# SophieLangdon27/LDPC_SPARC

Hardware: AMD Instinct MI355X
Metric: codewords/sec (AMP+BP) at L=1024 M=512 / n=1944; BER match vs CPU ref (higher is better)
Workload: dtype f32; 1 GPU; C2: SPARC AMP, regular design, sub-sampled DCT operator w=2^20; L=1024, M=512, n=6144, t_max=25, batch_per_gpu=256, parallelism=mc-shard x1 (independent codewords per GPU, RCCL all-reduce of error counters), counter_allreduce=none, engine=split per-codeword (amp_cw2.hip)

## Files before the change

### include/ldpc_sparc_amd.h

```cpp
#ifndef LDPC_SPARC_AMD_H
#define LDPC_SPARC_AMD_H

#include <stddef.h>
#include <stdint.h>

#ifdef __cplusplus
extern "C" {
#endif

enum sg_status {
    SG_OK = 0,
    SG_ERR_INVALID = -2,
    SG_ERR_BAD_ARG = SG_ERR_INVALID,
    SG_ERR_NO_DEVICE = -3,
    SG_ERR_HIP = -4,
    SG_ERR_NOMEM = -5,
    SG_ERR_UNSUPPORTED = -6,
    SG_ERR_COMM = -7
};

enum sg_dectype { SG_SUMPROD = 0, SG_SUMPROD2 = 1, SG_MINSUM = 2 };
enum sg_precision { SG_F64 = 0, SG_F32 = 1 };

const char *sg_last_error(void);
// ... 123 lines not shown
                          const double *alpha, const double *vk, const double *vk0, const double *tau2, int B,
                          int L, int M, double sqrt_nPl, double *out);

int sumprod(double *ch, long *vdeg, long *cdeg, long *intrlv, int Nv, int Nc, int Nmsg,
            double *app, int max_itcount);
int sumprod2(double *ch, long *vdeg, long *cdeg, long *intrlv, int Nv, int Nc, int Nmsg,
             double *app, int max_itcount);
int minsum(double *ch, long *vdeg, long *cdeg, long *intrlv, int Nv, int Nc, int Nmsg,
           double *app, double correction_factor, int max_itcount);
double Lxor(double L1, double L2, int corr_flag);
double Lxfb(double *L, long dc, int corr_flag);


typedef struct sg_amp_plan sg_amp_plan;

int sg_amp_plan_create(int ndim, const double *W, int Lr, int Lc, int L, int M, int n,
                       const uint32_t *order0, const uint32_t *order1, int precision,
                       sg_amp_plan **out);
int sg_amp_plan_destroy(sg_amp_plan *p);
int sg_amp_plan_info(const sg_amp_plan *p, int *w, int *nT, int *Mr, int *Mc, int *P, int *Q);
int sg_amp_plan_engine(const sg_amp_plan *p, int B);
int sg_amp_last_decode(const sg_amp_plan *p, int *engine, int *handover_iter, int *on_companion);
int sg_amp_plan_set_cus(sg_amp_plan *p, int cus);
int sg_amp_last_pipelined(const sg_amp_plan *p, int *pipelined);

int sg_amp_decode(sg_amp_plan *p, const double *y, int B, const int32_t *true_idx, double awgn_var,
                  int t_max, double rtol, int phi_method, int32_t *map_idx, int32_t *t_final,
                  double *nmse, double *psi);
int sg_amp_decode_device(sg_amp_plan *p, const void *d_y, int B, const int32_t *d_true_idx,
                         double awgn_var, int t_max, double rtol, int phi_method,
                         int32_t *d_map_idx, int32_t *d_t_final, double *d_nmse, double *d_psi,
                         void *stream);
int sg_amp_decode_partial_device(sg_amp_plan *p, const void *d_y, int B, const int32_t *d_known_idx,
                                 const int32_t *d_true_idx, double awgn_var, int t_max, double rtol,
                                 int phi_method, int32_t *d_map_idx, int32_t *d_t_final, double *d_nmse,
                                 double *d_psi, void *stream);
int sg_amp_decode_partial(sg_amp_plan *p, const double *y, int B, const int32_t *known_idx,
                          const int32_t *true_idx, double awgn_var, int t_max, double rtol, int phi_method,
                          int32_t *map_idx, int32_t *t_final, double *nmse, double *psi);
int sg_amp_decode_bpsk_device(sg_amp_plan *p, const void *d_y, int B, const int32_t *d_true_word, double awgn_var,
                              int t_max, double rtol, int phi_method, int32_t *d_map_word, int32_t *d_t_final,
                              double *d_nmse, double *d_psi, void *stream);
int sg_amp_decode_bpsk(sg_amp_plan *p, const double *y, int B, const int32_t *true_word, double awgn_var, int t_max,
                       double rtol, int phi_method, int32_t *map_word, int32_t *t_final, double *nmse, double *psi);
int sg_amp_decode_bpsk_partial_device(sg_amp_plan *p, const void *d_y, int B, const int32_t *d_known_word,
                                      const int32_t *d_true_word, double awgn_var, int t_max, double rtol,
// ... 91 lines not shown
```

### ldpc_sparc_amd/_native.py

```python
import ctypes as ct
import os

import numpy as np

_HERE = os.path.dirname(os.path.abspath(__file__))
LIB_PATH = os.environ.get("LDPC_SPARC_AMD_LIB", os.path.join(_HERE, "_lib", "libldpc_sparc_amd.so"))

SG_SUMPROD, SG_SUMPROD2, SG_MINSUM = 0, 1, 2
SG_F64, SG_F32 = 0, 1
SG_OK, SG_ERR_INVALID, SG_ERR_NO_DEVICE, SG_ERR_HIP, SG_ERR_NOMEM, SG_ERR_UNSUPPORTED, SG_ERR_COMM = 0, -2, -3, -4, -5, -6, -7
SG_ERR_BAD_ARG = SG_ERR_INVALID
DECTYPES = {"sumprod": SG_SUMPROD, "sumprod2": SG_SUMPROD2, "minsum": SG_MINSUM}

_lib = None

dp = ct.POINTER(ct.c_double)
lp = ct.POINTER(ct.c_long)
vp = ct.c_void_p


class NativeError(RuntimeError):
    pass


# ... 33 lines not shown
    ("sg_ldpc_decode_device", ct.c_int,
     [vp, ct.c_int, ct.c_int, vp, ct.c_int, ct.c_int, ct.c_double, vp, vp, vp]),
    ("sg_ldpc_layer_check", ct.c_int, [vp, vp, vp, ct.c_int, ct.c_int, ct.c_int, ct.c_int]),
    ("sg_ldpc_decode_layered", ct.c_int,
     [vp, ct.c_int, ct.c_int, ct.c_int, vp, ct.c_int, ct.c_int, ct.c_double, vp, vp]),
    ("sg_ldpc_decode_layered_device", ct.c_int,
     [vp, ct.c_int, ct.c_int, ct.c_int, vp, ct.c_int, ct.c_int, ct.c_double, vp, vp, vp]),
    ("sg_ldpc_decode_layered_kernel", ct.c_int, [vp, ct.c_int, ct.c_int, ct.c_int, ct.c_char_p, ct.c_size_t]),
    ("sg_ldpc_codeword_errors_device", ct.c_int, [vp, ct.c_int, vp, vp, ct.c_int, vp, vp]),
    ("sg_ldpc_count_errors_device", ct.c_int,
     [vp, ct.c_int, vp, vp, vp, ct.c_int, ct.c_int, vp, vp]),
    ("sumprod", ct.c_int, [dp, lp, lp, lp, ct.c_int, ct.c_int, ct.c_int, dp, ct.c_int]),
    ("sumprod2", ct.c_int, [dp, lp, lp, lp, ct.c_int, ct.c_int, ct.c_int, dp, ct.c_int]),
    ("minsum", ct.c_int, [dp, lp, lp, lp, ct.c_int, ct.c_int, ct.c_int, dp, ct.c_double, ct.c_int]),
    ("Lxor", ct.c_double, [ct.c_double, ct.c_double, ct.c_int]),
    ("sg_amp_plan_create", ct.c_int, [ct.c_int, vp, ct.c_int, ct.c_int, ct.c_int, ct.c_int, ct.c_int,
                                      vp, vp, ct.c_int, ct.POINTER(vp)]),
    ("sg_amp_plan_destroy", ct.c_int, [vp]),
    ("sg_amp_plan_info", ct.c_int, [vp] + [ct.POINTER(ct.c_int)] * 6),
    ("sg_amp_plan_engine", ct.c_int, [vp, ct.c_int]),
    ("sg_amp_last_decode", ct.c_int, [vp, ct.POINTER(ct.c_int), ct.POINTER(ct.c_int), ct.POINTER(ct.c_int)]),
    ("sg_amp_plan_set_cus", ct.c_int, [vp, ct.c_int]),
    ("sg_amp_last_pipelined", ct.c_int, [vp, ct.POINTER(ct.c_int)]),
    ("sg_amp_decode", ct.c_int, [vp, vp, ct.c_int, vp, ct.c_double, ct.c_int, ct.c_double, ct.c_int,
                                 vp, vp, vp, vp]),
    ("sg_amp_decode_device", ct.c_int, [vp, vp, ct.c_int, vp, ct.c_double, ct.c_int, ct.c_double,
                                        ct.c_int, vp, vp, vp, vp, vp]),
    ("sg_amp_decode_partial", ct.c_int, [vp, vp, ct.c_int, vp, vp, ct.c_double, ct.c_int, ct.c_double, ct.c_int,
                                         vp, vp, vp, vp]),
    ("sg_amp_decode_partial_device", ct.c_int, [vp, vp, ct.c_int, vp, vp, ct.c_double, ct.c_int, ct.c_double,
                                                ct.c_int, vp, vp, vp, vp, vp]),
    ("sg_concat_known_sections_device", ct.c_int, [ct.c_int, vp, vp, ct.c_int, ct.c_int, ct.c_int, ct.c_int, ct.c_int,
                                                   ct.c_int, ct.c_int, vp, vp]),
    ("sg_amp_decode_bpsk", ct.c_int, [vp, vp, ct.c_int, vp, ct.c_double, ct.c_int, ct.c_double, ct.c_int,
                                      vp, vp, vp, vp]),
    ("sg_amp_decode_bpsk_device", ct.c_int, [vp, vp, ct.c_int, vp, ct.c_double, ct.c_int, ct.c_double,
                                             ct.c_int, vp, vp, vp, vp, vp]),
    ("sg_amp_encode_bpsk_device", ct.c_int, [vp, vp, ct.c_int, vp, vp]),
    ("sg_amp_decode_bpsk_partial", ct.c_int, [vp, vp, ct.c_int, vp, vp, ct.c_double, ct.c_int, ct.c_double,
                                              ct.c_int, vp, vp, vp, vp]),
    ("sg_amp_decode_bpsk_partial_device", ct.c_int, [vp, vp, ct.c_int, vp, vp, ct.c_double, ct.c_int, ct.c_double,
                                                     ct.c_int, vp, vp, vp, vp, vp]),
    ("sg_amp_bpsk_soft_output", ct.c_int, [vp, ct.c_int]),
    ("sg_amp_bpsk_llr_device", ct.c_int, [vp, ct.c_int, ct.c_int, ct.c_int, ct.c_int, ct.c_int, vp, vp]),
    ("sg_amp_bpsk_llr", ct.c_int, [vp, ct.c_int, ct.c_int, ct.c_int, ct.c_int, vp]),
    ("sg_amp_llr_device", ct.c_int, [vp, ct.c_int, ct.c_int, ct.c_int, ct.c_int, ct.c_int, vp, vp]),
# ... 278 lines not shown
```

### ldpc_sparc_amd/csrc/amp.hpp

```cpp
#pragma once
#include "common.hpp"
#include "device_util.hpp"
#include "fft.hpp"

namespace sg {

constexpr int AMP_MAX_EPT = 32;

template <typename T>
struct AmpTables {
    int nT, w, N2, P, Q, log2P, log2Q, npairs;
    int L, M, LM, n, Lr, Lc, Mr, Mc, ndim;
    const int32_t *t_row, *t_col;
    const int32_t *col_ptr, *col_t;
    const int32_t *inmap;
    const int32_t *outslot;
    const int32_t *rp_ptr;
    const int32_t *rp_i;
    const uint32_t *rp_ab;
    const cx<T> *rp_c;
    const int32_t *gs_ptr;
    const int32_t *gs_loc;
    const int32_t *gs_i;
    const cx<T> *gs_c;
// ... 113 lines not shown
    int maxseg;
    float inv_n2;
    int img;
    const uint32_t *kt;
    const uint16_t *cmask;
    const int32_t *oa, *ob;
    const cx<float> *oc;
    const int32_t *gi;
    const cx<float> *gc;
    const int32_t *cls_ptr;
    const uint32_t *cls_ls;
    const int32_t *qpos;
    const uint16_t *seg;
    const cx<float> *stw;
    uint64_t *tprof;
};
size_t cw_lds_bytes(int img, int nslots);

constexpr int CW2_THREADS = 512;
constexpr int CW2_NP = 4;
constexpr int CW2_SLICE = 9216;
__host__ __device__ constexpr int c2pos(int i) { return i + (i >> 5); }
constexpr uint32_t CW2_TRASH = 2 * (8192 + 256) + 2048;
constexpr uint32_t CW_SELF = 1u << 23;
constexpr int CW_OFFSHIFT = 24;
__host__ __device__ constexpr int cw2_otp(int ot) { return (ot + 3) & ~3; }
template <int OT>
__device__ __forceinline__ void ld_slots(__amdgpu_buffer_rsrc_t r, int tl, uint32_t *out) {
    constexpr int OTP = cw2_otp(OT);
#pragma unroll
    for (int q = 0; q < OTP / 4; ++q) {
        const auto v = __builtin_amdgcn_raw_buffer_load_b128(r, 4 * OTP * tl, 16 * q, 0);
#pragma unroll
        for (int c = 0; c < 4; ++c)
            if (4 * q + c < OT) out[4 * q + c] = v[c];
    }
}
__host__ __device__ constexpr bool cw2_vz_tm(int ot) { return ot <= 12; }
struct Cw2Tables {
    int L, M, LM, n, N2, Q, Lblk, OT, maxcls;
    int np;
    float inv_n2;
    const uint32_t *cmask;
    const uint32_t *ka;
    const uint32_t *kat;
    const int32_t *oi;
    const float4 *cf;
    const float4 *gf = nullptr;
    const float2 *gm;
    const float4 *gmt;
    int sh_off;
    uint32_t m4n;
    float inv_4n;
    const int32_t *cls_ptr;
    const uint32_t *cls_ls;
    const uint32_t *cls2;
    const uint32_t *clsp;
    const uint32_t *clss;
    const int32_t *qpos;
    const uint16_t *seg;
    float *xr;
    const uint2 *rab = nullptr, *wab = nullptr;
    float *vz;
    float *ys, *zs;
    float4 *part;
    uint64_t *tprof;
};
int cw2_launch_iter(const Cw2Tables &tb, const RegBufs<float> &bf, const AmpScalars &sc, const AmpParams &pr, int t,
                    hipStream_t s, hipEvent_t after_ctrl = nullptr);
int cw2_launch_z_natural(const Cw2Tables &tb, const RegBufs<float> &bf, hipStream_t s);
struct Cw2dTables {
    int L, M, LM, n, N2, Q, Lblk, OT, maxcls;
    const uint32_t *cmask, *ka, *kat;
    const int32_t *oi;
    const double *cf;
    const double *gf;
    const double *sa;
    const double *twp;
    const int32_t *cls_ptr;
    const uint32_t *cls2;
    const int32_t *qpos;
    const uint16_t *seg;
    double *xr;
    double *vz;
    double *ys, *zs;
// ... 64 lines not shown
```

### ldpc_sparc_amd/csrc/amp_cw2.hip

```cpp
#include "amp.hpp"

namespace sg {
namespace {

constexpr int C2_T = CW2_THREADS;
constexpr int C2_LOG2P = 13, C2_P = 1 << C2_LOG2P, C2_EPT = C2_P / C2_T;
constexpr int C2_SC = 9;
constexpr int C2_NC = 2;
static_assert(C2_EPT == 16, "the transform is written for 16 values per thread");

constexpr int C2_PRIO_FFT = 0, C2_PRIO_REST = 1;
#define C2_SETPRIO(p) __builtin_amdgcn_s_setprio(p)

constexpr int C2_RC = 4;

constexpr double C2_LOG2E = 1.4426950408889634074;
__device__ __forceinline__ float c2_exp2(float x) { return __builtin_amdgcn_exp2f(x); }

__device__ __forceinline__ cx<float> c2_w(const Cw2Tables &tb, uint32_t j) {
    const float x = (float)(j & (uint32_t)(tb.N2 - 1)) * tb.inv_n2;
    return {__builtin_amdgcn_cosf(x), -__builtin_amdgcn_sinf(x)};
}

typedef float c2f __attribute__((ext_vector_type(2)));
// ... 54 lines not shown
    auto tw = [&](c2f x, float c, float s) -> c2f {
        return __builtin_elementwise_fma(x.yx, INV ? c2f{-s, s} : c2f{s, -s}, x * c2f{c, c});
    };
    y[1][1] = tw(y[1][1], c1, s1);
    y[1][2] = tw(y[1][2], r2, r2);
    y[1][3] = tw(y[1][3], s1, c1);
    y[2][1] = tw(y[2][1], r2, r2);
    y[2][2] = c2_mi<INV>(y[2][2]);
    y[2][3] = tw(y[2][3], -r2, r2);
    y[3][1] = tw(y[3][1], s1, c1);
    y[3][2] = tw(y[3][2], -r2, r2);
    y[3][3] = tw(y[3][3], -c1, -s1);
#pragma unroll
    for (int k1 = 0; k1 < 4; ++k1) {
        c2f v0 = y[0][k1], v1 = y[1][k1], v2 = y[2][k1], v3 = y[3][k1];
        c2_dft4<INV>(v0, v1, v2, v3);
        a[k1] = v0;
        a[k1 + 4] = v1;
        a[k1 + 8] = v2;
        a[k1 + 12] = v3;
    }
}

template <bool INV>
__device__ __forceinline__ void c2_stage0_r32(int tid, uint32_t msk) {
    const int l = tid & 63, H = l >> 5, w = tid >> 6, j = (w << 5) | (l & 31);
    c2f v[16];
    const c2lds *src = c2_at(j + w + 264 * 16 * H);
#pragma unroll
    for (int jj = 0; jj < 16; ++jj) v[jj] = src[264 * jj];
#pragma unroll
    for (int jj = 0; jj < 16; ++jj) {
        int mx = __builtin_amdgcn_sbfe((int)msk, 2 * jj, 1), my = __builtin_amdgcn_sbfe((int)msk, 2 * jj + 1, 1);
        asm volatile("" : "+v"(mx), "+v"(my));
        v[jj] = c2f{__uint_as_float(__float_as_uint(v[jj].x) & (uint32_t)mx),
                    __uint_as_float(__float_as_uint(v[jj].y) & (uint32_t)my)};
    }
#pragma unroll
    for (int jj = 0; jj < 8; ++jj) swap32(v[jj], v[jj + 8]);
    {
        constexpr float co[8] = {1.f, 0.98078528040323044913f, 0.92387953251128675613f, 0.83146961230254523708f,
                                 0.70710678118654752440f, 0.55557023301960222474f, 0.38268343236508977173f,
                                 0.19509032201612826785f};
        constexpr float si[8] = {0.f, 0.19509032201612826785f, 0.38268343236508977173f, 0.55557023301960222474f,
                                 0.70710678118654752440f, 0.83146961230254523708f, 0.92387953251128675613f,
                                 0.98078528040323044913f};
#pragma unroll
        for (int jj = 0; jj < 8; ++jj) {
            const c2f u = v[jj], x16 = v[jj + 8];
            v[jj] = u + x16;
            const c2f wf = c2f{co[jj], INV ? si[jj] : -si[jj]};
            const c2f w = H ? c2_mi<INV>(wf) : wf;
            v[jj + 8] = c2_mul(u - x16, w);
        }
    }
// ... 25 lines not shown
        const float x1 = (float)k * inv, x4 = (float)((4 * k) & (16 * NS - 1)) * inv;
        const c2f w1 = c2f{__builtin_amdgcn_cosf(x1), INV ? __builtin_amdgcn_sinf(x1) : -__builtin_amdgcn_sinf(x1)};
        const c2f w4 = c2f{__builtin_amdgcn_cosf(x4), INV ? __builtin_amdgcn_sinf(x4) : -__builtin_amdgcn_sinf(x4)};
        const c2f w2 = c2_mul(w1, w1), w3 = c2_mul(w2, w1), w8 = c2_mul(w4, w4), w12 = c2_mul(w8, w4);
        const c2f wb[3] = {w1, w2, w3}, wq[3] = {w4, w8, w12};
#pragma unroll
        for (int b = 1; b < 4; ++b) v[b] = c2_mul(v[b], wb[b - 1]);
#pragma unroll
        for (int q = 1; q < 4; ++q) {
            v[4 * q] = c2_mul(v[4 * q], wq[q - 1]);
#pragma unroll
            for (int b = 1; b < 4; ++b) v[4 * q + b] = c2_mul(v[4 * q + b], c2_mul(wq[q - 1], wb[b - 1]));
        }
    }
    c2_dft16<INV>(v);
    const int bo = ((j - k) << 4) + k;
    __syncthreads();
    c2lds *dst = c2_at(bo + (bo >> 5));
#pragma unroll
    for (int r = 0; r < 16; ++r) dst[(NS + NS / 32) * r] = v[r];
    __syncthreads();
}

template <bool INV>
__device__ __forceinline__ void c2_fft(int tid, uint32_t msk) {
    c2_stage0_r32<INV>(tid, msk);
    c2_stage_r16<INV, 5>(opaque(tid));
    c2_stage_r16<INV, 9>(opaque(tid));
}

}

#if !defined(C2_STAMPS) && defined(SG_DIAG)
#define C2_STAMPS 1
#endif
#ifndef C2_STAMPS
#define C2_STAMPS 0
#endif
#define C2_TP(k)                                                                                                \
    do {                                                                                                        \
        if (C2_STAMPS && tb.tprof && threadIdx.x == 0)                                                          \
            tb.tprof[(size_t)blockIdx.x * 64 + (k)] = __builtin_readcyclecounter();                             \
    } while (0)
#define C2_TPC(k)                          \
    do {                                   \
        if (m2 == h * Qh + 2) C2_TP(k);   \
    } while (0)

constexpr size_t C2_IMG_BYTES = (size_t)c2pos(C2_P) * 8;
constexpr size_t C2_CP_BYTES = C2_IMG_BYTES + 2 * 1024 * 4 + 16 + 15 * 32 * 8;
constexpr size_t C2_LDS_BYTES = C2_CP_BYTES + 4 * 72;
__device__ __forceinline__ const int *c2_stage_cp(unsigned char *smem, const Cw2Tables &tb, int tid) {
    int *cp = reinterpret_cast<int *>(smem + C2_CP_BYTES);
    for (int i = tid; i <= tb.Q; i += C2_T) cp[i] = tb.cls_ptr[i];
    return cp;
}
static_assert(C2_TW1 * 8 == C2_IMG_BYTES + 2 * 1024 * 4 + 16, "twiddle table after the trash slot");
static_assert(CW2_TRASH == (C2_IMG_BYTES + 2 * 1024 * 4) / 4, "trash slot after the staged statistics");
constexpr uint32_t C2_AZ_MI_BYTES = (uint32_t)C2_IMG_BYTES + 8;
static_assert(C2_AZ_MI_BYTES == 8u * (uint32_t)c2pos(C2_P) + 8, "behind row P of the r = 0 pair");
static_assert(C2_AZ_MI_BYTES + 1024 * 8 <= C2_TW1 * 8, "the staged statistics end before the stage twiddles");

constexpr int C2_SN = C2_NC * C2_SC;


template <int OT>
__global__ __launch_bounds__(C2_T, 4) void cw2_ab(Cw2Tables tb, RegBufs<float> bf) {
    extern __shared__ __attribute__((aligned(16))) unsigned char smem[];
    float *dr = reinterpret_cast<float *>(smem);
    c2f *sMI = reinterpret_cast<c2f *>(smem + C2_IMG_BYTES);
    const int h = blockIdx.x % tb.np, cw = blockIdx.x / tb.np, tid = threadIdx.x;
    if (!bf.active[cw]) return;
    C2_SETPRIO(C2_PRIO_REST);
    const size_t lb = (size_t)cw * tb.L;
    for (int l = tid; l < tb.L; l += C2_T) {
        sMI[l] = c2f{bf.stM[lb + l], bf.stI[lb + l]};
    }
    const float inv_tp = (float)(C2_LOG2E / bf.tau[cw]);
    const float *s = bf.s + (size_t)cw * tb.LM;
    cx<float> Ha[OT], Hb[OT];
#pragma unroll
    for (int j = 0; j < OT; ++j) Ha[j] = Hb[j] = {0.f, 0.f};
    const int Qh = tb.Q / tb.np;
    c2_tw1_init<false>(tid);
// ... 38 lines not shown
            for (int i = 0; i < C2_SN; ++i) {
                v[i] = buf_ldf(rs0, 4 * tl + 4 * i * C2_T, 0);
                e[i] = buf_ldu(re, 4 * tl, 4 * i * C2_T);
            }
        }
        const uint32_t cmk = tb.cmask[m2 * C2_T + tl];
        if (PL && m2 > h * Qh) {
            accumulate(m2 - 1, kapf);
            __syncthreads();
        }
        C2_TPC(8);
#pragma unroll
        for (int c = 0; c < C2_NC; ++c) {
#pragma unroll
            for (int i = c * C2_SC; i < (c + 1) * C2_SC; ++i) {
                const int sec = e[i] >> 16;
                dr[e[i] & 0xffffu] = c2_beta(v[i], sMI[sec], inv_tp);
            }
            C2_TPC(1 + c);
        }
        __syncthreads();
        C2_TPC(3);
        C2_SETPRIO(C2_PRIO_FFT);
        c2_fft<false>(tl, cmk);
        C2_SETPRIO(C2_PRIO_REST);
        C2_TPC(6);
        if constexpr (PL) acc_tables(opaque(tid), kapf);
    }
    {
        uint32_t ka[OT];
        acc_tables(opaque(tid), ka);
        accumulate((h + 1) * Qh - 1, ka);
    }
    C2_TP(11);
    float *xr = tb.xr + ((size_t)cw * tb.np + h) * OT * C2_T;
#pragma unroll
    for (int j = 0; j < OT; ++j) {
        const float4 c = tb.cf[j * C2_T + tid];
        xr[j * C2_T + tid] = (c.x * Ha[j].x - c.y * Ha[j].y) + (c.z * Hb[j].x - c.w * Hb[j].y);
    }
}

__device__ __forceinline__ double c2_block_sum(double v, double *red) {
    for (int o = 32; o > 0; o >>= 1) v += __shfl_xor(v, o, 64);
    const int lane = threadIdx.x & 63, wid = threadIdx.x >> 6;
    __syncthreads();
    if (lane == 0) red[wid] = v;
// ... 132 lines not shown
    const bool have_beta = t > 0;
    const double tv = bf.tau[cw];
    const float tau = (float)tv, inv_tau = (float)(C2_LOG2E / tv);
    const float inv_tp = have_beta ? (float)(C2_LOG2E / bf.tau_prev[cw]) : 0.f;
    const c2lds *sMI = (const c2lds *)(size_t)C2_AZ_MI_BYTES;
    if (have_beta)
        for (int l = tid; l < tb.L; l += C2_T)
            *(c2lds *)(size_t)(C2_AZ_MI_BYTES + 8u * (uint32_t)l) = c2f{bf.stM[lb + l], bf.stI[lb + l]};
    float *s = bf.s + (size_t)cw * tb.LM;
    constexpr int OTP = cw2_otp(OT);
    constexpr bool VZH = cw2_vz_tm(OT);
    const float *vz = tb.vz + (size_t)cw * (VZH ? OTP : 2 * OT) * C2_T;
    const int Lb = tb.Lblk;
    float Mr[2] = {-INFINITY, -INFINITY}, R1[2] = {0.f, 0.f}, R2[2] = {0.f, 0.f}, st[2] = {NAN, NAN};
    int jt[2] = {-1, -1};
#pragma unroll
    for (int k = 0; k < 2; ++k) {
        const int sec = tid + k * C2_T;
        if (bf.true_idx && sec < Lb) jt[k] = tb.qpos[sec * tb.M + bf.true_idx[lb + sec]];
    }
    const int Qh = tb.Q / tb.np;
    c2_tw1_init<true>(tid);
    const int *cpl = c2_stage_cp(smem, tb, tid);
    const uint32_t rmk0 = tb.cmask[tb.Q * C2_T + tid];
    __syncthreads();
    C2_TP(42);
    for (int m2 = h * Qh; m2 < (h + 1) * Qh; ++m2) {
        const int tl = opaque(tid);
        C2_TPC(32);
        const uint32_t rmk = (uint32_t)opaque((int)rmk0);
        const int q0 = uni(cpl[m2]), q1 = uni(cpl[m2 + 1]);
        const __amdgpu_buffer_rsrc_t rs = buf_rsrc(s + q0, 4 * (q1 - q0));
        constexpr bool EARLY = OT <= 12;
        float v[C2_SN];
        uint32_t e[C2_SN / 2];
        auto load_slice = [&]() {
            const __amdgpu_buffer_rsrc_t re = buf_rsrc(tb.clsp + (size_t)m2 * (CW2_SLICE / 2), 2 * CW2_SLICE);
#pragma unroll
            for (int i = 0; i < C2_SN / 2; ++i) {
                const uint32_t w = buf_ldu(re, 4 * tl, 4 * i * C2_T);
                e[i] = w;
            }
            if (have_beta) {
#pragma unroll
                for (int i = 0; i < C2_SN; ++i) v[i] = buf_ldf(rs, 4 * tl + 4 * i * C2_T, 0);
            }
        };
        {
            constexpr int CH = VZH ? OT : (OT + 1) / 2;
            const __amdgpu_buffer_rsrc_t rv2 = buf_rsrc(vz, 8 * OTP * C2_T),
                                         rk = buf_rsrc(VZH ? tb.kat : tb.ka, 4 * OTP * C2_T);
            uint32_t kall[VZH ? OT : 1];
            c2f vall[VZH ? OT : 1];
            if constexpr (VZH) {
                ld_slots<OT>(rk, tl, kall);
                const __amdgpu_buffer_rsrc_t rv = buf_rsrc(vz, 4 * OTP * C2_T), rg = buf_rsrc(tb.gmt, 8 * OTP * C2_T);
                float v1[OTP];
#pragma unroll
                for (int q = 0; q < OTP / 4; ++q) {
                    const auto w = __builtin_amdgcn_raw_buffer_load_b128(rv, 4 * OTP * tl, 16 * q, 0);
#pragma unroll
                    for (int c = 0; c < 4; ++c) v1[4 * q + c] = __uint_as_float(w[c]);
                }
#pragma unroll
                for (int q = 0; q < OTP / 2; ++q) {
                    const auto w = __builtin_amdgcn_raw_buffer_load_b128(rg, 8 * OTP * tl, 16 * q, 0);
                    if (2 * q < OT)
                        vall[2 * q] = c2f{__uint_as_float(w[0]), __uint_as_float(w[1])} * v1[2 * q];
                    if (2 * q + 1 < OT)
                        vall[2 * q + 1] = c2f{__uint_as_float(w[2]), __uint_as_float(w[3])} * v1[2 * q + 1];
                }
            }
            const uint32_t cm = 3u + 8u * (uint32_t)m2;
            c2f u0{0.f, 0.f}, u1{0.f, 0.f};
#pragma unroll
            for (int j0 = 0; j0 < OT; j0 += CH) {
                uint32_t ka[CH];
                c2f vv[CH];
#pragma unroll
                for (int i = 0; i < CH; ++i) {
                    const int j = j0 + i < OT ? j0 + i : OT - 1;
                    if constexpr (VZH) {
                        ka[i] = kall[j];
                        vv[i] = vall[j];
                    } else {
                        ka[i] = buf_ldu(rk, 4 * tl, 4 * j * C2_T);
                        const auto w = __builtin_amdgcn_raw_buffer_load_b64(rv2, 8 * tl, 8 * j * C2_T, 0);
                        vv[i] = c2f{__uint_as_float(w[0]), __uint_as_float(w[1])};
                    }
                }
#pragma unroll
                for (int j = 0; j < CH; ++j) {
                    if (j0 + j >= OT) break;
                    const uint32_t k = ka[j];
// ... 12 lines not shown
                    u1 = __builtin_elementwise_fma(cs.yx, vv[j].yy, u1 * keep);
                    const uint32_t r = k & (uint32_t)(C2_P - 1), rb = (uint32_t)C2_P - r;
                    c2lds *pa = (c2lds *)(size_t)(8u * (r + (r >> 5))), *pb = (c2lds *)(size_t)(8u * (rb + (rb >> 5)));
                    *pb = u1;
                    *pa = __builtin_elementwise_fma(u1, c2f{selff, selff}, u0);
                }
            }
        }
        if constexpr (EARLY) load_slice();
        int sa[2], sb[2];
        {
            const __amdgpu_buffer_rsrc_t rg = buf_rsrc(tb.seg + (size_t)m2 * (Lb + 1), 2 * (Lb + 1));
#pragma unroll
            for (int k = 0; k < 2; ++k) {
                const int sec = tl + k * C2_T;
                sa[k] = __builtin_amdgcn_raw_buffer_load_b16(rg, 2 * sec, 0, 0);
                sb[k] = __builtin_amdgcn_raw_buffer_load_b16(rg, 2 * sec + 2, 0, 0);
            }
        }
        C2_TPC(33);
        __syncthreads();
        C2_TPC(34);
        C2_SETPRIO(C2_PRIO_FFT);
        c2_fft<true>(tl, rmk);
        C2_SETPRIO(C2_PRIO_REST);
        C2_TPC(35);
        float snv[C2_SN];
        if constexpr (!EARLY) load_slice();
        if (have_beta) {
            uint32_t es[C2_SN / 2];
            const __amdgpu_buffer_rsrc_t rc = buf_rsrc(tb.clss + (size_t)m2 * (CW2_SLICE / 2), 2 * CW2_SLICE);
#pragma unroll
            for (int i = 0; i < C2_SN / 2; ++i) es[i] = buf_ldu(rc, 4 * tl, 4 * i * C2_T);
#pragma unroll
            for (int c = 0; c < C2_NC; ++c) {
                float u[C2_SC];
#pragma unroll
                for (int i = 0; i < C2_SC; ++i) u[i] = dr[c ? e[i] >> 16 : e[i] & 0xffffu];
#pragma unroll
                for (int i = 0; i < C2_SC; ++i) {
                    const uint32_t sec = c ? es[i] >> 16 : es[i] & 0xffffu;
                    snv[c * C2_SC + i] = __builtin_fmaf(u[i], tau, c2_beta(v[c * C2_SC + i], sMI[sec], inv_tp));
                }
                __builtin_amdgcn_sched_barrier(0);
            }
        } else {
#pragma unroll
// ... 185 lines not shown
        ProfScope ps(SG_PH_CW2_AB, s);
        hipLaunchKernelGGL((cw2_ab<OT>), g2, dim3(C2_T), lds, s, tb, bf);
    }
    {
        ProfScope ps(SG_PH_CW2_CTRL, s);
        hipLaunchKernelGGL((cw2_ctrl<OT>), gB, dim3(C2_T), 0, s, tb, bf, sc, pr, t);
    }
    if (after_ctrl) SG_HIP(hipEventRecord(after_ctrl, s));
    {
        ProfScope ps(SG_PH_CW2_AZ, s);
        hipLaunchKernelGGL((cw2_az<OT>), g2, dim3(C2_T), lds, s, tb, bf, t);
    }
    {
        ProfScope ps(SG_PH_CW2_CTRL, s);
        hipLaunchKernelGGL((cw2_merge), gB, dim3(1024), 0, s, tb, bf, sc, pr, t);
    }
    return SG_OK;
}

int cw2_launch_iter(const Cw2Tables &tb, const RegBufs<float> &bf, const AmpScalars &sc, const AmpParams &pr, int t,
                    hipStream_t s, hipEvent_t after_ctrl) {
    if (bf.B <= 0) return SG_OK;
    if (tb.Q % 2 || tb.L > 1024 || tb.Lblk > 2 * C2_T || tb.maxcls > C2_NC * C2_SC * C2_T ||
        fpad(tb.maxcls + 16) >= 2 * C2_P || tb.N2 != C2_P * tb.Q)
        return fail(SG_ERR_UNSUPPORTED, "split per-codeword engine: sizes outside its compile-time bounds");
    ProfScope ps(SG_PH_AMP_CW, s);
    switch (tb.OT) {
    case 12: SG_TRY(cw2_launch<12>(tb, bf, sc, pr, t, s, after_ctrl)); break;
    case 13: SG_TRY(cw2_launch<13>(tb, bf, sc, pr, t, s, after_ctrl)); break;
    case 14: SG_TRY(cw2_launch<14>(tb, bf, sc, pr, t, s, after_ctrl)); break;
    case 16: SG_TRY(cw2_launch<16>(tb, bf, sc, pr, t, s, after_ctrl)); break;
    default: return fail(SG_ERR_UNSUPPORTED, "split per-codeword engine: %d outputs per thread", tb.OT);
    }
    SG_HIP(hipGetLastError());
    return SG_OK;
}

}
```

### ldpc_sparc_amd/csrc/amp_plan.hpp

```cpp
#pragma once
#include <algorithm>
#include <complex>
#include <cstdlib>
#include <cstring>
#include <cmath>
#include <vector>

#include "amp.hpp"
#include "amp_oploop.hpp"
#include "device_mem.hpp"
#include "integ_ws.hpp"

using cd = std::complex<double>;

struct sg_amp_plan {
    int precision = SG_F32;
    sg_amp_plan *last_ran = nullptr;
    int last_engine = -1, last_handover = -1;
    int last_B = 0;
    int device = 0;
    int ndim = 0, L = 0, M = 0, LM = 0, n = 0, Lr = 1, Lc = 1, Mr = 0, Mc = 0, nT = 0;
    int w = 0, N2 = 0, P = 0, Q = 0, log2P = 0, log2Q = 0, npairs = 0;
    std::vector<double> W;
    sg::DevPool tables;
// ... 26 lines not shown
    int32_t *h_active = nullptr; int h_active_cap = 0;
    hipEvent_t poll_ev = nullptr;
    hipStream_t pipe_stream = nullptr;
    hipEvent_t pipe_ev[4] = {nullptr, nullptr, nullptr, nullptr};
    int cus_assumed = 0;
    int last_piped = 0;
    void *ws_s = nullptr, *ws_tu = nullptr, *ws_xn = nullptr, *ws_part = nullptr, *ws_stM = nullptr,
         *ws_stI = nullptr;
    double *ws_tau_prev = nullptr;
    bool cw = false;
    int cwKT = 0;
    bool no_cw = false;
    sg_amp_plan *alt = nullptr;
    uint32_t *c_kt = nullptr;
    uint16_t *c_cmask = nullptr;
    int32_t *c_oa = nullptr, *c_ob = nullptr, *c_gi = nullptr;
    void *c_gc = nullptr, *c_stw = nullptr;
    int cw2OT = 0;
    int c2_np = 2;
    uint32_t *c2_ka = nullptr, *c2_kat = nullptr, *c2_cmask = nullptr, *c2_cls = nullptr, *c2_clsp = nullptr,
             *c2_clss = nullptr;
    int32_t *c2_oi = nullptr;
    void *c2_cf = nullptr;
    float *c2_gm = nullptr;
    float *c2_gmt = nullptr;
    int c2_shoff = 0;
    double *c2d_cf = nullptr, *c2d_gf = nullptr, *c2d_sa = nullptr, *c2d_twp = nullptr;
    void *ws_c2xp = nullptr, *ws_c2vz = nullptr, *ws_c2part = nullptr, *ws_c2ys = nullptr, *ws_c2zs = nullptr;
    void *ws_c2beta = nullptr, *ws_c2sec = nullptr;
    bool block = false;
    bool block2 = false;
    int b2_log2p = 0;
    int32_t *b_gk = nullptr;
    uint16_t *b_gloc = nullptr;
    uint32_t *b_pos2 = nullptr, *b_oab = nullptr;
    int32_t *b_gptr = nullptr, *b_gi = nullptr, *b_grow = nullptr;
    int b_ngs = 0;
    void *ws_gbuf = nullptr;
    void *b_oc = nullptr, *b_gc = nullptr, *b_stw = nullptr;
    sg::IntegWs wi;
    sg::DevPool wp;
    int cap_Bp = 0;
    void *wp_u = nullptr, *wp_r = nullptr, *wp_z = nullptr;
    double *wp_zz = nullptr, *wp_bsq = nullptr, *wp_err = nullptr, *wp_tau = nullptr;
    int32_t *wp_active = nullptr, *wp_known = nullptr;
    bool bpsk_soft = false;
// ... 67 lines not shown
```

### ldpc_sparc_amd/csrc/amp_plan_cw.cpp

```cpp
#include <random>

#include "amp_plan.hpp"

namespace sg {

template <typename Len, typename Cell>
static void bank_balance(std::vector<std::vector<int>> &own, int KT, Len len_of, Cell cell) {
    const int T = (int)own.size();
    std::vector<int> at((size_t)T * KT, -1), pos((size_t)T * KT, -1), start((size_t)T * KT, 0);
    for (int t = 0; t < T; ++t) {
        int j = 0;
        for (int i = 0; i < (int)own[t].size(); ++i) {
            const int r = own[t][i], len = len_of(r);
            start[(size_t)t * KT + j] = len;
            for (int q = 0; q < len; ++q, ++j) {
                at[(size_t)t * KT + j] = r;
                pos[(size_t)t * KT + j] = i;
            }
        }
    }
    std::vector<std::vector<int>> by((size_t)KT * (KT + 1));
    for (int t = 0; t < T; ++t)
        for (int j = 0; j < KT; ++j)
            if (const int len = start[(size_t)t * KT + j]) by[(size_t)j * (KT + 1) + len].push_back(t);
// ... 247 lines not shown
                ka[c] = e;
                oi[c] = i;
                last_word[tid] = e & ~(CW_VALID | CW_NEWROW);
                const float v[4] = {(float)o.c1.real(), (float)o.c1.imag(), (float)o.c2.real(), (float)o.c2.imag()};
                std::copy(v, v + 4, cf.begin() + 4 * c);
                if (f64) {
                    const double d[8] = {o.c1.real(), o.c1.imag(), o.c2.real(), o.c2.imag(),
                                         o.al.real(), o.al.imag(), o.be.real(), o.be.imag()};
                    std::copy(d, d + 4, cfd.begin() + 4 * c);
                    std::copy(d + 4, d + 8, gfd.begin() + 4 * c);
                    const cd w = tw(o.a, N2);
                    sad[2 * c] = w.real();
                    sad[2 * c + 1] = w.imag();
                }
            }
        }
    }
    if (p->precision != SG_F64)
        for (int tid = 0; tid < T; ++tid)
            for (int j = 0; j < OT; ++j) {
                uint32_t &e = ka[(size_t)j * T + tid];
                if (!(e & CW_VALID)) e = last_word[tid];
            }
    std::vector<uint32_t> cmask((size_t)(Q + 1) * T, 0u);
    auto mbit = [&](int m2, int m1, int c) {
        const int j = m1 & 255, g = m1 >> 8;
        const int tid = ((j >> 5) << 6) | ((g >> 4) << 5) | (j & 31);
        cmask[(size_t)m2 * T + tid] |= 1u << (2 * (g & 15) + c);
    };
    for (int m2 = 0; m2 < Q; ++m2)
        for (int q = cls_ptr[m2]; q < cls_ptr[m2 + 1]; ++q) {
            const int loc = (int)(cls_ls[q] & 0xffffu);
            mbit(m2, fsw(loc >> 1), loc & 1);
        }
    for (int r : row_k1) {
        mbit(Q, r, 0);
        mbit(Q, r, 1);
    }
    std::vector<uint32_t> cls2((size_t)Q * CW2_SLICE, CW2_TRASH);
    for (int m2 = 0; m2 < Q; ++m2)
        for (int q = cls_ptr[m2]; q < cls_ptr[m2 + 1]; ++q) {
            const uint32_t loc = cls_ls[q] & 0xffffu;
            const uint32_t pl = 2u * (uint32_t)c2pos(fsw((int)(loc >> 1))) + (loc & 1u);
            cls2[(size_t)m2 * CW2_SLICE + (q - cls_ptr[m2])] = (cls_ls[q] & ~0xffffu) | pl;
        }
    SG_TRY(p->tables.upload(&p->c2_cls, cls2));
    {
        constexpr int H = CW2_SLICE / 2;
        std::vector<uint32_t> clsp((size_t)Q * H), clss((size_t)Q * H);
        for (int m2 = 0; m2 < Q; ++m2)
            for (int q = 0; q < H; ++q) {
                const uint32_t *c = &cls2[(size_t)m2 * CW2_SLICE];
                clsp[(size_t)m2 * H + q] = (c[q] & 0xffffu) | (c[q + H] << 16);
                clss[(size_t)m2 * H + q] = (c[q] >> 16) | (c[q + H] & ~0xffffu);
            }
        SG_TRY(p->tables.upload(&p->c2_clsp, clsp));
        if (!f64) SG_TRY(p->tables.upload(&p->c2_clss, clss));
    }
    SG_TRY(p->tables.upload(&p->c2_cmask, cmask));
    SG_TRY(p->tables.upload(&p->c2_ka, ka));
    {
        const int OTP = cw2_otp(OT);
        std::vector<uint32_t> kat((size_t)OTP * T, 0u);
        for (int tid = 0; tid < T; ++tid)
            for (int j = 0; j < OT; ++j) kat[(size_t)tid * OTP + j] = ka[(size_t)j * T + tid];
        SG_TRY(p->tables.upload(&p->c2_kat, kat));
    }
    SG_TRY(p->tables.upload(&p->c2_oi, oi));
    SG_TRY(p->tables.upload((float **)&p->c2_cf, cf));
    SG_TRY(p->tables.upload(&p->c2_gm, gm));
    {
        const int OTP = cw2_otp(OT);
        std::vector<float> gmt((size_t)OTP * T * 2, 0.f);
        for (int tid = 0; tid < T; ++tid)
            for (int j = 0; j < OT; ++j)
                for (int c = 0; c < 2; ++c) gmt[((size_t)tid * OTP + j) * 2 + c] = gm[((size_t)j * T + tid) * 2 + c];
        SG_TRY(p->tables.upload(&p->c2_gmt, gmt));
    }
    p->c2_shoff = pow2 ? ilog2((int)(N / 2)) : 0;
    if (f64) {
        std::vector<double> twp((size_t)P * 2);
        for (int k = 0; k < P; ++k) {
// ... 11 lines not shown
}

CwTables ctables(const sg_amp_plan *p, int B) {
    CwTables tb;
    tb.L = p->L; tb.M = p->M; tb.LM = p->LM; tb.n = p->n; tb.N2 = p->N2; tb.Q = p->rQ; tb.Lblk = p->Lblk;
    tb.KT = p->cwKT; tb.log2P = p->rlog2P; tb.maxcls = p->rmaxcls; tb.maxseg = p->rmaxseg;
    tb.img = p->rimg;
    tb.cmask = p->c_cmask;
    tb.kt = p->c_kt; tb.oa = p->c_oa; tb.ob = p->c_ob; tb.oc = (const cx<float> *)p->r_oc;
    tb.gi = p->c_gi; tb.gc = (const cx<float> *)p->c_gc;
    tb.cls_ptr = p->r_cls_ptr; tb.cls_ls = p->r_cls_ls; tb.qpos = p->r_qpos; tb.seg = p->r_seg;
    tb.stw = (const cx<float> *)p->c_stw;
    tb.inv_n2 = 1.0f / (float)p->N2;
    tb.tprof = p->tprof_items * 20 >= (size_t)32 * B ? p->tprof.at<uint64_t>() : nullptr;
    return tb;
}

Cw2Tables c2tables(const sg_amp_plan *p, int B) {
    Cw2Tables tb;
    tb.L = p->L; tb.M = p->M; tb.LM = p->LM; tb.n = p->n; tb.N2 = p->N2; tb.Q = p->rQ; tb.Lblk = p->Lblk;
    tb.OT = p->cw2OT; tb.maxcls = p->rmaxcls;
    tb.np = p->c2_np >= 4 && CW2_NP >= 4 && p->rQ % 4 == 0 ? 4 : 2;
    tb.inv_n2 = 1.0f / (float)p->N2;
    tb.cmask = p->c2_cmask; tb.ka = p->c2_ka; tb.kat = p->c2_kat; tb.oi = p->c2_oi;
    tb.cf = (const float4 *)p->c2_cf; tb.gm = (const float2 *)p->c2_gm;
    tb.gmt = (const float4 *)p->c2_gmt;
    tb.sh_off = p->c2_shoff; tb.m4n = (uint32_t)(4 * p->w - 1); tb.inv_4n = (float)(1.0 / (4.0 * (double)p->w));
    tb.cls_ptr = p->r_cls_ptr; tb.cls_ls = p->r_cls_ls; tb.cls2 = p->c2_cls; tb.clsp = p->c2_clsp; tb.clss = p->c2_clss;
    tb.qpos = p->r_qpos; tb.seg = p->r_seg;
    tb.xr = (float *)p->ws_c2xp; tb.vz = (float *)p->ws_c2vz; tb.ys = (float *)p->ws_c2ys; tb.zs = (float *)p->ws_c2zs; tb.part = (float4 *)p->ws_c2part;
    tb.tprof = p->tprof_items * 20 >= (size_t)64 * tb.np * B ? p->tprof.at<uint64_t>() : nullptr;
    return tb;
}

Cw2dTables c2dtables(const sg_amp_plan *p) {
    Cw2dTables tb;
    tb.L = p->L; tb.M = p->M; tb.LM = p->LM; tb.n = p->n; tb.N2 = p->N2; tb.Q = p->rQ; tb.Lblk = p->Lblk;
    tb.OT = p->cw2OT; tb.maxcls = p->rmaxcls;
    tb.cmask = p->c2_cmask; tb.ka = p->c2_ka; tb.kat = p->c2_kat; tb.oi = p->c2_oi;
    tb.cf = p->c2d_cf; tb.gf = p->c2d_gf; tb.sa = p->c2d_sa; tb.twp = p->c2d_twp;
    tb.cls_ptr = p->r_cls_ptr; tb.cls2 = p->c2_cls; tb.qpos = p->r_qpos; tb.seg = p->r_seg;
    tb.xr = (double *)p->ws_c2xp; tb.vz = (double *)p->ws_c2vz; tb.ys = (double *)p->ws_c2ys;
    tb.zs = (double *)p->ws_c2zs; tb.beta = (double *)p->ws_c2beta; tb.sec = (double *)p->ws_c2sec;
    return tb;
}

}
```

Baseline: 13750 codewords/s.

## Zero stale image rows explicitly instead of masking inverse FFT stage0 input

```diff
diff --git a/include/ldpc_sparc_amd.h b/include/ldpc_sparc_amd.h
--- a/include/ldpc_sparc_amd.h
+++ b/include/ldpc_sparc_amd.h
@@ -169,6 +169,7 @@
 int sg_amp_plan_engine(const sg_amp_plan *p, int B);
 int sg_amp_last_decode(const sg_amp_plan *p, int *engine, int *handover_iter, int *on_companion);
 int sg_amp_plan_set_cus(sg_amp_plan *p, int cus);
+int sg_amp_plan_cw2_rows(const sg_amp_plan *p, int *written, int *zeroed, int *both, int *neither, int *per_thread);
 int sg_amp_last_pipelined(const sg_amp_plan *p, int *pipelined);
 
 int sg_amp_decode(sg_amp_plan *p, const double *y, int B, const int32_t *true_idx, double awgn_var,
diff --git a/ldpc_sparc_amd/_native.py b/ldpc_sparc_amd/_native.py
--- a/ldpc_sparc_amd/_native.py
+++ b/ldpc_sparc_amd/_native.py
@@ -79,6 +79,7 @@
     ("sg_amp_last_decode", ct.c_int, [vp, ct.POINTER(ct.c_int), ct.POINTER(ct.c_int), ct.POINTER(ct.c_int)]),
     ("sg_amp_plan_set_cus", ct.c_int, [vp, ct.c_int]),
     ("sg_amp_last_pipelined", ct.c_int, [vp, ct.POINTER(ct.c_int)]),
+    ("sg_amp_plan_cw2_rows", ct.c_int, [vp] + [ct.POINTER(ct.c_int)] * 5),
     ("sg_amp_decode", ct.c_int, [vp, vp, ct.c_int, vp, ct.c_double, ct.c_int, ct.c_double, ct.c_int,
                                  vp, vp, vp, vp]),
     ("sg_amp_decode_device", ct.c_int, [vp, vp, ct.c_int, vp, ct.c_double, ct.c_int, ct.c_double,
diff --git a/ldpc_sparc_amd/csrc/amp.hpp b/ldpc_sparc_amd/csrc/amp.hpp
--- a/ldpc_sparc_amd/csrc/amp.hpp
+++ b/ldpc_sparc_amd/csrc/amp.hpp
@@ -159,6 +159,9 @@
 constexpr int CW2_SLICE = 9216;
 __host__ __device__ constexpr int c2pos(int i) { return i + (i >> 5); }
 constexpr uint32_t CW2_TRASH = 2 * (8192 + 256) + 2048;
+constexpr uint32_t CW2_ZTRASH = (4 * CW2_TRASH + 8) / 8;
+static_assert(CW2_TRASH % 2 == 0 && CW2_ZTRASH < (1u << 16), "zrow packs 8-byte-aligned addresses / 8 in 16 bits");
+constexpr int CW2_ZRW = 8;
 constexpr uint32_t CW_SELF = 1u << 23;
 constexpr int CW_OFFSHIFT = 24;
 __host__ __device__ constexpr int cw2_otp(int ot) { return (ot + 3) & ~3; }
@@ -178,6 +181,7 @@
     int L, M, LM, n, N2, Q, Lblk, OT, maxcls;
     int np;
     float inv_n2;
+    int zrw;
     const uint32_t *cmask;
     const uint32_t *ka;
     const uint32_t *kat;
@@ -197,7 +201,8 @@
     const int32_t *qpos;
     const uint16_t *seg;
     float *xr;
-    const uint2 *rab = nullptr, *wab = nullptr;
+    const uint32_t *zrow;
+    const uint2 *wab = nullptr;
     float *vz;
     float *ys, *zs;
     float4 *part;
diff --git a/ldpc_sparc_amd/csrc/amp_cw2.hip b/ldpc_sparc_amd/csrc/amp_cw2.hip
--- a/ldpc_sparc_amd/csrc/amp_cw2.hip
+++ b/ldpc_sparc_amd/csrc/amp_cw2.hip
@@ -100,7 +100,7 @@
     }
 }
 
-template <bool INV>
+template <bool INV, bool MASKED>
 __device__ __forceinline__ void c2_stage0_r32(int tid, uint32_t msk) {
     const int l = tid & 63, H = l >> 5, w = tid >> 6, j = (w << 5) | (l & 31);
     c2f v[16];
@@ -108,7 +108,7 @@
 #pragma unroll
     for (int jj = 0; jj < 16; ++jj) v[jj] = src[264 * jj];
 #pragma unroll
-    for (int jj = 0; jj < 16; ++jj) {
+    for (int jj = 0; MASKED && jj < 16; ++jj) {
         int mx = __builtin_amdgcn_sbfe((int)msk, 2 * jj, 1), my = __builtin_amdgcn_sbfe((int)msk, 2 * jj + 1, 1);
         asm volatile("" : "+v"(mx), "+v"(my));
         v[jj] = c2f{__uint_as_float(__float_as_uint(v[jj].x) & (uint32_t)mx),
@@ -180,9 +180,9 @@
     __syncthreads();
 }
 
-template <bool INV>
+template <bool INV, bool MASKED>
 __device__ __forceinline__ void c2_fft(int tid, uint32_t msk) {
-    c2_stage0_r32<INV>(tid, msk);
+    c2_stage0_r32<INV, MASKED>(tid, msk);
     c2_stage_r16<INV, 5>(opaque(tid));
     c2_stage_r16<INV, 9>(opaque(tid));
 }
@@ -218,6 +218,8 @@
 constexpr uint32_t C2_AZ_MI_BYTES = (uint32_t)C2_IMG_BYTES + 8;
 static_assert(C2_AZ_MI_BYTES == 8u * (uint32_t)c2pos(C2_P) + 8, "behind row P of the r = 0 pair");
 static_assert(C2_AZ_MI_BYTES + 1024 * 8 <= C2_TW1 * 8, "the staged statistics end before the stage twiddles");
+static_assert(C2_AZ_MI_BYTES + 1024 * 8 == 8 * CW2_ZTRASH && 8 * CW2_ZTRASH + 8 == C2_TW1 * 8,
+              "zrow's padding between cw2_az's staged statistics and the stage twiddles");
 
 constexpr int C2_SN = C2_NC * C2_SC;
 
@@ -302,7 +304,7 @@
         __syncthreads();
         C2_TPC(3);
         C2_SETPRIO(C2_PRIO_FFT);
-        c2_fft<false>(tl, cmk);
+        c2_fft<false, true>(tl, cmk);
         C2_SETPRIO(C2_PRIO_REST);
         C2_TPC(6);
         if constexpr (PL) acc_tables(opaque(tid), kapf);
@@ -481,13 +483,11 @@
     const int Qh = tb.Q / tb.np;
     c2_tw1_init<true>(tid);
     const int *cpl = c2_stage_cp(smem, tb, tid);
-    const uint32_t rmk0 = tb.cmask[tb.Q * C2_T + tid];
     __syncthreads();
     C2_TP(42);
     for (int m2 = h * Qh; m2 < (h + 1) * Qh; ++m2) {
         const int tl = opaque(tid);
         C2_TPC(32);
-        const uint32_t rmk = (uint32_t)opaque((int)rmk0);
         const int q0 = uni(cpl[m2]), q1 = uni(cpl[m2 + 1]);
         const __amdgpu_buffer_rsrc_t rs = buf_rsrc(s + q0, 4 * (q1 - q0));
         constexpr bool EARLY = OT <= 12;
@@ -509,10 +509,20 @@
             constexpr int CH = VZH ? OT : (OT + 1) / 2;
             const __amdgpu_buffer_rsrc_t rv2 = buf_rsrc(vz, 8 * OTP * C2_T),
                                          rk = buf_rsrc(VZH ? tb.kat : tb.ka, 4 * OTP * C2_T);
+            const int zrw = tb.zrw;
+            const __amdgpu_buffer_rsrc_t rz = buf_rsrc(tb.zrow, 4 * zrw * C2_T);
+            auto zero_rows = [](uint32_t w0, uint32_t w1) {
+                *(c2lds *)(size_t)((w0 & 0xffffu) << 3) = c2f{0.f, 0.f};
+                *(c2lds *)(size_t)((w0 >> 16) << 3) = c2f{0.f, 0.f};
+                *(c2lds *)(size_t)((w1 & 0xffffu) << 3) = c2f{0.f, 0.f};
+                *(c2lds *)(size_t)((w1 >> 16) << 3) = c2f{0.f, 0.f};
+            };
             uint32_t kall[VZH ? OT : 1];
             c2f vall[VZH ? OT : 1];
             if constexpr (VZH) {
+                const auto zw = __builtin_amdgcn_raw_buffer_load_b64(rz, 4 * zrw * tl, 0, 0);
                 ld_slots<OT>(rk, tl, kall);
+                zero_rows(zw[0], zw[1]);
                 const __amdgpu_buffer_rsrc_t rv = buf_rsrc(vz, 4 * OTP * C2_T), rg = buf_rsrc(tb.gmt, 8 * OTP * C2_T);
                 float v1[OTP];
 #pragma unroll
@@ -529,6 +539,11 @@
                     if (2 * q + 1 < OT)
                         vall[2 * q + 1] = c2f{__uint_as_float(w[2]), __uint_as_float(w[3])} * v1[2 * q + 1];
                 }
+            }
+#pragma unroll 1
+            for (int q = VZH ? 2 : 0; q < zrw; q += 2) {
+                const auto zq = __builtin_amdgcn_raw_buffer_load_b64(rz, 4 * zrw * tl, 4 * q, 0);
+                zero_rows(zq[0], zq[1]);
             }
             const uint32_t cm = 3u + 8u * (uint32_t)m2;
             c2f u0{0.f, 0.f}, u1{0.f, 0.f};
@@ -587,7 +602,7 @@
         __syncthreads();
         C2_TPC(34);
         C2_SETPRIO(C2_PRIO_FFT);
-        c2_fft<true>(tl, rmk);
+        c2_fft<true, false>(tl, 0u);
         C2_SETPRIO(C2_PRIO_REST);
         C2_TPC(35);
         float snv[C2_SN];
@@ -819,7 +834,8 @@
                     hipStream_t s, hipEvent_t after_ctrl) {
     if (bf.B <= 0) return SG_OK;
     if (tb.Q % 2 || tb.L > 1024 || tb.Lblk > 2 * C2_T || tb.maxcls > C2_NC * C2_SC * C2_T ||
-        fpad(tb.maxcls + 16) >= 2 * C2_P || tb.N2 != C2_P * tb.Q)
+        fpad(tb.maxcls + 16) >= 2 * C2_P || tb.N2 != C2_P * tb.Q || tb.zrw < 2 || tb.zrw % 2 ||
+        tb.zrw > CW2_ZRW || !tb.zrow)
         return fail(SG_ERR_UNSUPPORTED, "split per-codeword engine: sizes outside its compile-time bounds");
     ProfScope ps(SG_PH_AMP_CW, s);
     switch (tb.OT) {
diff --git a/ldpc_sparc_amd/csrc/amp_plan.hpp b/ldpc_sparc_amd/csrc/amp_plan.hpp
--- a/ldpc_sparc_amd/csrc/amp_plan.hpp
+++ b/ldpc_sparc_amd/csrc/amp_plan.hpp
@@ -72,6 +72,8 @@
              *c2_clss = nullptr;
     int32_t *c2_oi = nullptr;
     void *c2_cf = nullptr;
+    uint32_t *c2_zrow = nullptr;
+    int c2_zrw = 0;
     float *c2_gm = nullptr;
     float *c2_gmt = nullptr;
     int c2_shoff = 0;
diff --git a/ldpc_sparc_amd/csrc/amp_plan_cw.cpp b/ldpc_sparc_amd/csrc/amp_plan_cw.cpp
--- a/ldpc_sparc_amd/csrc/amp_plan_cw.cpp
+++ b/ldpc_sparc_amd/csrc/amp_plan_cw.cpp
@@ -293,6 +293,35 @@
                 uint32_t &e = ka[(size_t)j * T + tid];
                 if (!(e & CW_VALID)) e = last_word[tid];
             }
+    int zrw = 0;
+    std::vector<uint32_t> zrow;
+    if (!f64) {
+        std::vector<uint8_t> written(P, 0), needed(P, 0);
+        for (uint32_t e : ka) {
+            const int r = (int)(e & (uint32_t)(P - 1));
+            written[r] = 1;
+            if (r) written[P - r] = 1;
+        }
+        for (int r : row_k1) {
+            if (r < 0 || r >= P) return SG_OK;
+            needed[r] = 1;
+        }
+        std::vector<int> stale;
+        for (int m1 = 0; m1 < P; ++m1) {
+            if (written[m1] != needed[m1]) return SG_OK;
+            if (!needed[m1]) stale.push_back(m1);
+        }
+        const int ZR = ((int)stale.size() + T - 1) / T;
+        zrw = std::max(2, (ZR + 3) / 4 * 2);
+        if (zrw > CW2_ZRW) return SG_OK;
+        zrow.assign((size_t)zrw * T, CW2_ZTRASH | (CW2_ZTRASH << 16));
+        for (size_t i = 0; i < stale.size(); ++i) {
+            const int tid = (int)(i % T), k = (int)(i / T);
+            uint32_t &wd = zrow[(size_t)tid * zrw + k / 2];
+            const uint32_t a = (uint32_t)c2pos(stale[i]);
+            wd = k % 2 ? (wd & 0xffffu) | (a << 16) : (wd & ~0xffffu) | a;
+        }
+    }
     std::vector<uint32_t> cmask((size_t)(Q + 1) * T, 0u);
     auto mbit = [&](int m2, int m1, int c) {
         const int j = m1 & 255, g = m1 >> 8;
@@ -329,6 +358,8 @@
         if (!f64) SG_TRY(p->tables.upload(&p->c2_clss, clss));
     }
     SG_TRY(p->tables.upload(&p->c2_cmask, cmask));
+    if (!f64) SG_TRY(p->tables.upload(&p->c2_zrow, zrow));
+    p->c2_zrw = zrw;
     SG_TRY(p->tables.upload(&p->c2_ka, ka));
     {
         const int OTP = cw2_otp(OT);
@@ -386,6 +417,7 @@
     tb.OT = p->cw2OT; tb.maxcls = p->rmaxcls;
     tb.np = p->c2_np >= 4 && CW2_NP >= 4 && p->rQ % 4 == 0 ? 4 : 2;
     tb.inv_n2 = 1.0f / (float)p->N2;
+    tb.zrw = p->c2_zrw; tb.zrow = p->c2_zrow;
     tb.cmask = p->c2_cmask; tb.ka = p->c2_ka; tb.kat = p->c2_kat; tb.oi = p->c2_oi;
     tb.cf = (const float4 *)p->c2_cf; tb.gm = (const float2 *)p->c2_gm;
     tb.gmt = (const float4 *)p->c2_gmt;
@@ -396,6 +428,59 @@
     tb.tprof = p->tprof_items * 20 >= (size_t)64 * tb.np * B ? p->tprof.at<uint64_t>() : nullptr;
     return tb;
 }
+
+}
+
+extern "C" int sg_amp_plan_cw2_rows(const sg_amp_plan *p, int *written, int *zeroed, int *both, int *neither,
+                                    int *per_thread) {
+    using namespace sg;
+    SG_CHECK_ARG(p, "plan is NULL");
+    SG_CHECK_ARG(p->precision != SG_F64 && p->cw2OT && p->c2_ka && p->c2_zrow,
+                 "the plan has no f32 split per-codeword engine");
+    const int P = p->rP, T = CW2_THREADS;
+    const int zrw = p->c2_zrw;
+    std::vector<uint32_t> ka((size_t)p->cw2OT * T), zrow((size_t)zrw * T);
+    SG_HIP(hipMemcpy(ka.data(), p->c2_ka, ka.size() * sizeof(uint32_t), hipMemcpyDeviceToHost));
+    if (!zrow.empty()) SG_HIP(hipMemcpy(zrow.data(), p->c2_zrow, zrow.size() * sizeof(uint32_t), hipMemcpyDeviceToHost));
+    std::vector<int> wr(P, 0), zr(P, 0), at(c2pos(P), -1);
+    for (int m1 = 0; m1 < P; ++m1) at[c2pos(m1)] = m1;
+    for (uint32_t e : ka) {
+        const int r = (int)(e & (uint32_t)(P - 1));
+        wr[r] = 1;
+        if (r) wr[P - r] = 1;
+    }
+    int per = 0, bad = 0;
+    for (int tid = 0; tid < T; ++tid) {
+        int mine = 0;
+        for (int q = 0; q < zrw; ++q)
+            for (uint32_t a : {zrow[(size_t)tid * zrw + q] & 0xffffu, zrow[(size_t)tid * zrw + q] >> 16}) {
+                if (a == CW2_ZTRASH) continue;
+                if (a >= (uint32_t)c2pos(P) || at[a] < 0) {
+                    ++bad;
+                    continue;
+                }
+                ++zr[at[a]];
+                ++mine;
+            }
+        per = std::max(per, mine);
+    }
+    SG_CHECK_ARG(!bad, "internal: %d zeroed addresses outside the image's rows", bad);
+    int nw = 0, nz = 0, nb = 0, nn = 0;
+    for (int m1 = 0; m1 < P; ++m1) {
+        nw += wr[m1];
+        nz += zr[m1];
+        nb += wr[m1] && zr[m1];
+        nn += !wr[m1] && !zr[m1];
+    }
+    if (written) *written = nw;
+    if (zeroed) *zeroed = nz;
+    if (both) *both = nb;
+    if (neither) *neither = nn;
+    if (per_thread) *per_thread = per;
+    return SG_OK;
+}
+
+namespace sg {
 
 Cw2dTables c2dtables(const sg_amp_plan *p) {
     Cw2dTables tb;
```

New measurement: 13880 codewords/s, median of 6. Within noise of the previous version (+0.9%).
